# Cornell-RelaxML/QuIP

Hardware: NVIDIA H100
Metric: tokens/sec 2-bit Llama-2-7B (per-layer eval path, seq 2048) (higher is better)
Workload: dtype f16

## Files before the change

quip_b200/csrc/api.cu:

```cuda
#include <stdarg.h>
#include <string.h>

#include <vector>

#include "common.cuh"

namespace quip {

static thread_local char g_err[512] = "";
std::atomic<int64_t> g_launches{0};

void set_error(const char* fmt, ...) {
  va_list ap;
  va_start(ap, fmt);
  vsnprintf(g_err, sizeof(g_err), fmt, ap);
  va_end(ap);
}

int qgemm_skinny(const QuipLinearDesc* d, const __half* x, const __half* bias, __half* z, int M, int ksplit,
                 float* part, int* counters, cudaStream_t s);
int skinny_pick_ksplit(int N, int K, int rows_per_cta, int M);
size_t skinny_workspace_bytes(int N, int M, int ksplit);
int qgemv(const QuipLinearDesc* d, const __half* x, const __half* bias, __half* z, int M, cudaStream_t s);
bool qgemv_fits(int K, int M, int bits);
int qgemm_tc(const QuipLinearDesc* d, const __half* x, const float* xsum, const __half* bias, __half* z, int M,
             cudaStream_t s);

extern int g_gather_rows, g_pass_min_tiles, g_fewtok;
extern int g_fewtok_max_m;
bool side_fused_ok(const QuipSide* sd, int n);
int side_fused(const QuipSide* sd, const __half* in, __half* out, int64_t M, const int32_t* in_idx, const float* in_scale,
               const int32_t* out_idx, const __half* out_bias, float* xsum, cudaStream_t s);
bool pass_fewtok_ok(const QuipPass* ps, int64_t M, int n);
int pass_fewtok(const QuipPass* ps, const __half* in, __half* out, int64_t M, int n, const int32_t* in_idx,
                const float* in_scale, const int32_t* out_inv, const __half* out_bias, cudaStream_t s);
extern int g_gv_rbc, g_gv_persist, g_gv_int, g_gv_tma, g_gv_cw, g_gv_stream;
bool side_fewtok_ok(const QuipSide* sd, int n, int64_t M);
int side_fewtok(const QuipSide* sd, const __half* in, __half* out, int64_t M, int n, const int32_t* in_idx,
                const float* in_scale, const int32_t* out_inv, const __half* out_bias, cudaStream_t s);

static int g_side_fused = 1;
static int g_pdl = 1;
static int g_use_gemv = 1;
static int g_sk_ksplit = 0;
static int g_side_fewtok = 0;

int launch_pdl(const void* kern, dim3 grid, dim3 block, size_t smem, cudaStream_t s, void** args) {
  cudaLaunchConfig_t cfg = {};
  cfg.gridDim = grid;
  cfg.blockDim = block;
  cfg.dynamicSmemBytes = smem;
  cfg.stream = s;
  cudaLaunchAttribute attr[1];
  attr[0].id = cudaLaunchAttributeProgrammaticStreamSerialization;
  attr[0].val.programmaticStreamSerializationAllowed = 1;
  cfg.attrs = attr;
  cfg.numAttrs = g_pdl ? 1 : 0;
  cudaError_t e = cudaLaunchKernelExC(&cfg, kern, args);
  if (e != cudaSuccess) {
    cudaGetLastError();
    set_error("kernel launch failed: %s", cudaGetErrorString(e));
    return QUIP_ERR_CUDA;
  }
  return QUIP_OK;
}

constexpr size_t WS_HEADER = 16 * 1024;
constexpr int SKINNY_MAX_M = 32;

static size_t align_up(size_t v, size_t a) { return (v + a - 1) / a * a; }

struct WsPlan {
  size_t xsum, bufA, bufB, zbuf, bufC, part, total;
};
// ... 12 lines not shown
  p.bufB = off; if (v_on) off += xk;
  p.zbuf = off; if (u_on) off += xn;
  p.bufC = off; if (u_on) off += xn;
  p.part = off;
  const int mc = M <= SKINNY_MAX_M ? (int)M : SKINNY_MAX_M;
  off += align_up(skinny_workspace_bytes(d->N, mc, skinny_pick_ksplit(d->N, d->K, 64, mc)), 256);
  p.total = off;
  return p;
}

static int check_desc(const QuipLinearDesc* d) {
  QUIP_CHECK_ARG(d != nullptr, "null descriptor");
  QUIP_CHECK_ARG(d->bits >= 2 && d->bits <= 4, "bits must be 2, 3 or 4 (got %d)", d->bits);
  QUIP_CHECK_ARG(d->K > 0 && d->K % 128 == 0, "K=%d must be a positive multiple of 128", d->K);
  QUIP_CHECK_ARG(d->N > 0 && d->N % 16 == 0, "N=%d must be a positive multiple of 16", d->N);
  QUIP_CHECK_ARG(d->qweight && d->scales && d->zeros, "qweight / scales / zeros must be set");
  QUIP_CHECK_ARG(d->V.n == 0 || d->V.n == d->K, "V side size %d != K %d", d->V.n, d->K);
  QUIP_CHECK_ARG(d->U.n == 0 || d->U.n == d->N, "U side size %d != N %d", d->U.n, d->N);
  QUIP_CHECK_ARG(d->V.npass >= 0 && d->V.npass <= 2 && d->U.npass >= 0 && d->U.npass <= 2, "npass must be 0..2");
  return QUIP_OK;
}

struct TimedLaunch {
  cudaEvent_t e0, e1;
  int path;
  double flops, bytes;
};
static bool g_timing = false;
static std::vector<TimedLaunch> g_timed;
static std::vector<TimedLaunch> g_pool;
constexpr size_t TIMED_MAX = 1 << 16;

static int run_qgemm_untimed(const QuipLinearDesc* d, const __half* x2, const float* xsum, const __half* bias,
                             __half* z, int64_t M, int path, unsigned char* ws, const WsPlan& p, cudaStream_t s);

static int run_qgemm(const QuipLinearDesc* d, const __half* x2, const float* xsum, const __half* bias, __half* z,
                     int64_t M, int path, unsigned char* ws, const WsPlan& p, cudaStream_t s) {
  if (path == 0)
    path = M <= SKINNY_MAX_M ? 1 : 2;
  if (!g_timing || g_timed.size() >= TIMED_MAX) return run_qgemm_untimed(d, x2, xsum, bias, z, M, path, ws, p, s);
  TimedLaunch t;
  if (!g_pool.empty()) {
    t = g_pool.back();
    g_pool.pop_back();
  } else {
    QUIP_CUDA(cudaEventCreate(&t.e0));
    QUIP_CUDA(cudaEventCreate(&t.e1));
  }
  t.path = path;
  t.flops = 2.0 * (double)M * d->N * d->K;
  t.bytes = (double)d->N * d->K * d->bits / 8.0 + 2.0 * (double)M * (d->K + d->N);
  QUIP_CUDA(cudaEventRecord(t.e0, s));
  int e = run_qgemm_untimed(d, x2, xsum, bias, z, M, path, ws, p, s);
  QUIP_CUDA(cudaEventRecord(t.e1, s));
  g_timed.push_back(t);
  return e;
}

static int run_qgemm_untimed(const QuipLinearDesc* d, const __half* x2, const float* xsum, const __half* bias,
                             __half* z, int64_t M, int path, unsigned char* ws, const WsPlan& p, cudaStream_t s) {
  if (path == 1) {
    for (int64_t m0 = 0; m0 < M; m0 += SKINNY_MAX_M) {
      int mc = (int)((M - m0) < SKINNY_MAX_M ? (M - m0) : SKINNY_MAX_M);
      if (g_use_gemv && qgemv_fits(d->K, mc, d->bits)) {
        if (int e = qgemv(d, x2 + m0 * d->K, bias, z + m0 * d->N, mc, s)) return e;
        continue;
      }
      int ksplit = skinny_pick_ksplit(d->N, d->K, 64, mc);
      if (g_sk_ksplit > 0 && g_sk_ksplit < ksplit) ksplit = g_sk_ksplit;
      if (int e = qgemm_skinny(d, x2 + m0 * d->K, bias, z + m0 * d->N, mc, ksplit,
                               reinterpret_cast<float*>(ws + p.part), reinterpret_cast<int*>(ws), s))
        return e;
    }
    return QUIP_OK;
  }
  const bool need_xsum = !(d->flags & QUIP_FLAG_SYMMETRIC);
  QUIP_CHECK_ARG(!need_xsum || xsum, "asymmetric grid needs the row sums of x");
  return qgemm_tc(d, x2, xsum, bias, z, (int)M, s);
}

}

using namespace quip;

extern "C" const char* quip_last_error(void) { return g_err; }
extern "C" int quip_abi_version(void) { return QUIP_ABI_VERSION; }
extern "C" int64_t quip_launch_count(void) { return g_launches.load(); }

extern "C" int quip_config(const char* key, int value) {
  QUIP_CHECK_ARG(key != nullptr, "null key");
  if (!strcmp(key, "side_fused")) { g_side_fused = value; return QUIP_OK; }
  if (!strcmp(key, "side_fewtok")) { g_side_fewtok = value; return QUIP_OK; }
  if (!strcmp(key, "pdl")) { g_pdl = value; return QUIP_OK; }
  if (!strcmp(key, "fewtok")) { g_fewtok = value; return QUIP_OK; }
  if (!strcmp(key, "fewtok_max_m")) {
    QUIP_CHECK_ARG(value >= 8 && value <= 32, "quip_config: fewtok_max_m must be in 8..32");
    g_fewtok_max_m = value;
    return QUIP_OK;
  }
  if (!strcmp(key, "gemv")) { g_use_gemv = value; return QUIP_OK; }
  if (!strcmp(key, "gv_rbc")) { g_gv_rbc = value; return QUIP_OK; }
  if (!strcmp(key, "gv_stream")) { g_gv_stream = value; return QUIP_OK; }
  if (!strcmp(key, "gv_cw")) { g_gv_cw = value; return QUIP_OK; }
  if (!strcmp(key, "gv_tma")) { g_gv_tma = value; return QUIP_OK; }
  if (!strcmp(key, "gv_int")) { g_gv_int = value; return QUIP_OK; }
  if (!strcmp(key, "gv_persist")) { g_gv_persist = value; return QUIP_OK; }
  if (!strcmp(key, "gather_rows")) { g_gather_rows = value; return QUIP_OK; }
  if (!strcmp(key, "sk_ksplit")) { g_sk_ksplit = value; return QUIP_OK; }
  if (!strcmp(key, "pass_min_tiles")) { g_pass_min_tiles = value > 0 ? value : 1; return QUIP_OK; }
  set_error("quip_config: unknown key '%s'", key);
  return QUIP_ERR_ARG;
}

extern "C" int quip_timing_enable(int on) {
  g_timing = on != 0;
  return QUIP_OK;
}
extern "C" int quip_timing_reset(void) {
  for (auto& t : g_timed) g_pool.push_back(t);
  g_timed.clear();
  return QUIP_OK;
}
extern "C" int quip_timing_read(int path, double* total_ms, int64_t* launches, double* flops, double* bytes) {
  double ms = 0, fl = 0, by = 0;
// ... 1 lines not shown
  for (auto& t : g_timed) {
    if (t.path != path) continue;
    QUIP_CUDA(cudaEventSynchronize(t.e1));
    float dt = 0.f;
    QUIP_CUDA(cudaEventElapsedTime(&dt, t.e0, t.e1));
    ms += dt; fl += t.flops; by += t.bytes; ++n;
  }
  if (total_ms) *total_ms = ms;
  if (launches) *launches = n;
  if (flops) *flops = fl;
  if (bytes) *bytes = by;
  return QUIP_OK;
}

extern "C" int quip_qlinear_workspace_bytes(const QuipLinearDesc* d, int64_t M, size_t* out) {
  if (int e = check_desc(d)) return e;
  QUIP_CHECK_ARG(out && M > 0, "bad arguments");
  *out = plan_ws(d, M).total;
  return QUIP_OK;
}

extern "C" int quip_qgemm(const QuipLinearDesc* d, const void* x2, const float* xsum, const void* bias, void* z,
                          int64_t M, int path, void* workspace, size_t workspace_bytes, void* stream) {
  if (int e = check_desc(d)) return e;
  QUIP_CHECK_ARG(x2 && z && M > 0 && M < (1ll << 31), "bad arguments");
  WsPlan p = plan_ws(d, M);
  QUIP_CHECK_ARG(path >= 0 && path <= 2, "path must be 0 (auto), 1 (few-token kernels) or 2 (tensor-core GEMM)");
  if (path == 1 || (path == 0 && M <= SKINNY_MAX_M)) {
    if (!workspace || workspace_bytes < p.total) {
      set_error("workspace too small: need %zu bytes, have %zu", p.total, workspace_bytes);
      return QUIP_ERR_WORKSPACE;
    }
  }
  return run_qgemm(d, (const __half*)x2, xsum, (const __half*)bias, (__half*)z, M, path, (unsigned char*)workspace, p,
                   (cudaStream_t)stream);
}

extern "C" int quip_qlinear_forward(const QuipLinearDesc* d, const void* x_, void* y_, int64_t M, void* workspace,
                                    size_t workspace_bytes, void* stream) {
  if (int e = check_desc(d)) return e;
  QUIP_CHECK_ARG(x_ && y_ && M > 0 && M < (1ll << 31), "bad arguments");
  cudaStream_t s = (cudaStream_t)stream;
  WsPlan p = plan_ws(d, M);
  if (!workspace || workspace_bytes < p.total) {
    set_error("workspace too small: need %zu bytes, have %zu", p.total, workspace_bytes);
    return QUIP_ERR_WORKSPACE;
  }
  unsigned char* ws = (unsigned char*)workspace;
  const __half* x = (const __half*)x_;
  __half* y = (__half*)y_;
  __half* bufA = (__half*)(ws + p.bufA);
  __half* bufB = (__half*)(ws + p.bufB);
  __half* zbuf = (__half*)(ws + p.zbuf);
  __half* bufC = (__half*)(ws + p.bufC);
  float* xsum = (float*)(ws + p.xsum);
  const int K = d->K, N = d->N;

  const __half* cur = x;
  const int vpass = d->V.n ? d->V.npass : 0;
  const bool need_xsum = !(d->flags & QUIP_FLAG_SYMMETRIC) && M > SKINNY_MAX_M;
  bool have_xsum = false;
  if (g_fewtok && g_side_fewtok && vpass == 2 && side_fewtok_ok(&d->V, K, M)) {
    if (int e = side_fewtok(&d->V, x, bufA, M, K, d->V.idx, d->inv_scale, nullptr, nullptr, s)) return e;
    cur = bufA;
  } else if (g_side_fused && M > g_fewtok_max_m && vpass == 2 && side_fused_ok(&d->V, K)) {
    if (int e = side_fused(&d->V, x, bufA, M, d->V.idx, d->inv_scale, nullptr, nullptr, need_xsum ? xsum : nullptr, s)) return e;
    cur = bufA;
    have_xsum = need_xsum;
  } else {
    const bool fuse_in = g_fewtok && M <= g_fewtok_max_m && vpass > 0 && d->V.pass[0].p <= 128 && pass_fewtok_ok(&d->V.pass[0], M, K);
    if ((d->V.idx || d->inv_scale) && !fuse_in) {
      if (int e = quip_gather(cur, bufA, M, K, d->V.n ? d->V.idx : nullptr, d->inv_scale, nullptr, stream)) return e;
      cur = bufA;
    }
    for (int i = 0; i < vpass; ++i) {
      __half* dst = (cur == bufA) ? bufB : bufA;
      if (i == 0 && fuse_in) {
        if (int e = pass_fewtok(&d->V.pass[0], cur, dst, M, K, d->V.idx, d->inv_scale, nullptr, nullptr, s)) return e;
      } else if (int e = quip_rot_pass(&d->V.pass[i], cur, dst, M, K, 0, stream)) {
        return e;
      }
      cur = dst;
    }
  }
  const __half* x2 = cur;

  const bool u_on = side_on(d->U);
  if (need_xsum && !have_xsum)
    if (int e = quip_rowsum(x2, xsum, M, K, stream)) return e;
  __half* zdst = u_on ? zbuf : y;
  if (int e = run_qgemm(d, x2, xsum, u_on ? nullptr : (const __half*)d->bias, zdst, M, 0, ws, p, s)) return e;
  if (!u_on) return QUIP_OK;

  if (g_fewtok && g_side_fewtok && d->U.npass == 2 && (!d->U.idx || d->U.inv_idx) && side_fewtok_ok(&d->U, N, M))
    return side_fewtok(&d->U, zbuf, y, M, N, nullptr, nullptr, d->U.inv_idx, (const __half*)d->bias, s);
  if (g_side_fused && M > g_fewtok_max_m && d->U.npass == 2 && side_fused_ok(&d->U, N))
    return side_fused(&d->U, zbuf, y, M, nullptr, nullptr, d->U.idx, (const __half*)d->bias, nullptr, s);
  const __half* zc = zbuf;
  const int np = d->U.npass;
  bool tail_gather = d->U.idx || d->bias;
  const bool fuse_out = tail_gather && g_fewtok && M <= g_fewtok_max_m && np > 0 && (!d->U.idx || d->U.inv_idx) &&
                        pass_fewtok_ok(&d->U.pass[np - 1], M, N);
  if (fuse_out) tail_gather = false;
  for (int i = 0; i < np; ++i) {
    __half* dst = (i == np - 1 && !tail_gather) ? y : ((zc == zbuf) ? bufC : zbuf);
    if (i == np - 1 && fuse_out) {
      if (int e = pass_fewtok(&d->U.pass[i], zc, dst, M, N, nullptr, nullptr, d->U.inv_idx, (const __half*)d->bias, s)) return e;
    } else if (int e = quip_rot_pass(&d->U.pass[i], zc, dst, M, N, 0, stream)) {
      return e;
    }
    zc = dst;
  }
  if (tail_gather) return quip_gather(zc, y, M, N, d->U.idx, nullptr, d->bias, stream);
  return QUIP_OK;
}
```

quip_b200/csrc/qgemm_tc.cu:

```cuda
#include "tc_common.cuh"

namespace quip {

constexpr int TC_SMEM_MAX = 227 * 1024;

template <int BITS, int BN, bool DENSE>
struct TcCfg {
  static constexpr int A_BYTES = DENSE ? TC_BM * TC_BK * 2 : (TC_BM / SB_ROWS) * sb_words(BITS) * 4;
  static constexpr int B_BYTES = BN * TC_BK * 2;
  static constexpr int STAGE_BYTES = A_BYTES + B_BYTES;
  static constexpr int EPI_HALVES = BN * 72 > 64 * (BN + 8) ? BN * 72 : 64 * (BN + 8);
  static constexpr int EPI_BYTES = 2 * EPI_HALVES * 2;
  static constexpr int STAGES_FIT = (TC_SMEM_MAX - EPI_BYTES - 1024 - 256) / STAGE_BYTES;
  static constexpr int STAGES = STAGES_FIT < 16 ? STAGES_FIT : 16;
  static constexpr size_t SMEM = (size_t)STAGES * STAGE_BYTES + 1024  + 256  + EPI_BYTES;
  static_assert(STAGE_BYTES % 1024 == 0 && 2 * STAGES * 8 <= 256, "stage layout");
};

template <int BITS, int BN, bool DENSE>
__global__ void __launch_bounds__(TC_THREADS, 1)
qgemm_tc_kernel(const __grid_constant__ CUtensorMap tmap_x, const __grid_constant__ CUtensorMap tmap_a,
                const float* __restrict__ scales, const float* __restrict__ zeros, const __half* __restrict__ bias,
                const float* __restrict__ xsum, __half* __restrict__ z, int M, int K, int N, int symmetric, int nblk,
                int shared_factor) {
  using C = TcCfg<BITS, BN, DENSE>;
  extern __shared__ unsigned char smem_raw[];
  const uint32_t smem_base = (smem_u32(smem_raw) + 1023u) & ~1023u;
  unsigned char* smem_gen = smem_raw + (smem_base - smem_u32(smem_raw));
  uint64_t* bars = reinterpret_cast<uint64_t*>(smem_gen + (size_t)C::STAGES * C::STAGE_BYTES);
  uint64_t* full = bars;
  uint64_t* empty = bars + C::STAGES;
  __half* epi = reinterpret_cast<__half*>(smem_gen + (size_t)C::STAGES * C::STAGE_BYTES + 256);

  const int warp = threadIdx.x >> 5, lane = threadIdx.x & 31;
  const int tiles_n = DENSE ? (N + BN - 1) / BN : (N + TC_BM - 1) / TC_BM;
  const int tiles_m = DENSE ? (M + TC_BM - 1) / TC_BM : (M + BN - 1) / BN;
  const int per_blk = tiles_n * tiles_m;
  const int num_tiles = per_blk * nblk;
  const int KB = (K + TC_BK - 1) / TC_BK;
  const int64_t ldz = (int64_t)N * nblk;
  constexpr int TMA_WARP = TC_CONSUMER_WARPS;

  if (warp == TMA_WARP && lane == 0) {
    asm volatile("prefetch.tensormap [%0];" ::"l"(&tmap_x) : "memory");
    asm volatile("prefetch.tensormap [%0];" ::"l"(&tmap_a) : "memory");
    for (int s = 0; s < C::STAGES; ++s) {
      mbar_init(&full[s], 1);
      mbar_init(&empty[s], TC_CONSUMER_WARPS);
    }
    asm volatile("fence.mbarrier_init.release.cluster;" ::: "memory");
  }
  __syncthreads();

  if (warp == TMA_WARP) {
    if (lane == 0) {
      int s = 0;
      uint32_t ph = 0;
// ... 21 lines not shown
    const int wg = warp >> 2, wtid = threadIdx.x & 127;
    const int frow = (warp & 3) * 16 + (lane >> 2);
    const int fcol = (lane & 3) * 2;
    __half* eb = epi + wg * C::EPI_HALVES;
    float acc[BN / 2];
#pragma unroll
    for (int j = 0; j < BN / 2; ++j) acc[j] = 0.f;
    int s = 0;
    uint32_t ph = 0;
    auto advance = [&]() { if (++s == C::STAGES) { s = 0; ph ^= 1u; } };
    auto release = [&](int st) {
      __syncwarp();
      if (lane == 0) mbar_arrive(&empty[st]);
    };
    for (int tile = blockIdx.x; tile < num_tiles; tile += gridDim.x) {
      const int blk = tile / per_blk, rr = tile % per_blk;
      int prev = 0;
      const int n_base = (rr % tiles_n) * TC_BM + wg * 64, m0 = (rr / tiles_n) * BN;
      float Pn[2], Rn[2], bn[2];
      if constexpr (!DENSE) {
#pragma unroll
        for (int h = 0; h < 2; ++h) {
          const int n = n_base + frow + 8 * h;
          Pn[h] = 1.f; Rn[h] = 0.f; bn[h] = 0.f;
          if (n < N) {
            const float sc = scales[n];
            Pn[h] = sc * (float)(1 << BITS);
            if (!symmetric) Rn[h] = sc * (0.5f * (float)((1 << BITS) - 1)) - zeros[n];
            if (bias) bn[h] = __half2float(bias[n]);
          }
        }
        if (!symmetric && wtid < BN / 32 && m0 + 32 * wtid < M)
          asm volatile("prefetch.global.L1 [%0];" ::"l"(xsum + m0 + 32 * wtid));
      }
      if constexpr (DENSE) {
        for (int kb = 0; kb < KB; ++kb) {
          mbar_wait(&full[s], ph);
          const uint32_t a_addr = smem_base + (uint32_t)(s * C::STAGE_BYTES);
          const uint64_t adesc = make_sw128_desc(a_addr + (uint32_t)(wg * 64 * 128));
          const uint64_t bdesc = make_sw128_desc(a_addr + C::A_BYTES);
          wgmma_fence();
#pragma unroll
          for (int k = 0; k < TC_BK / 16; ++k)
            wgmma_f16_ss<BN>(acc, adesc + (uint64_t)(2 * k), bdesc + (uint64_t)(2 * k), (kb | k) ? 1 : 0);
          wgmma_commit();
          wgmma_wait<1>();
          if (kb > 0) release(prev);
          prev = s;
          advance();
        }
      } else {
        const int g = lane >> 2, t = lane & 3;
        const uint32_t row_off = (uint32_t)(warp * sb_words(BITS) * 4);
        uint32_t w[row_words(BITS)];
        uint32_t fa[2][16];
        auto issue = [&](const uint32_t (&f)[16], int first) {
          const uint64_t bdesc = make_sw128_desc(smem_base + (uint32_t)(s * C::STAGE_BYTES) + C::A_BYTES);
          wgmma_fence();
#pragma unroll
          for (int k = 0; k < TC_BK / 16; ++k)
            wgmma_f16_rs<BN>(acc, &f[4 * k], bdesc + (uint64_t)(2 * k), (first && k == 0) ? 0 : 1);
          wgmma_commit();
        };
        auto load_words = [&]() {
          mbar_wait(&full[s], ph);
          tc_load_row_words<BITS>(smem_base + (uint32_t)(s * C::STAGE_BYTES) + row_off, g, w);
// ... 21 lines not shown
          prev = s;
          advance();
          if (ksb + 1 < KSB) {
            load_words();
            frag_natural<BITS, 0, 0>(w, t, &fa[0][0]);
            frag_natural<BITS, 0, 1>(w, t, &fa[0][4]);
            frag_natural<BITS, 1, 0>(w, t, &fa[0][8]);
            frag_natural<BITS, 1, 1>(w, t, &fa[0][12]);
          }
        }
      }
      wgmma_wait<0>();
      wgmma_fence_regs(acc);
      release(prev);

      if constexpr (DENSE) {
        constexpr int EP = BN + 8;
#pragma unroll
        for (int j = 0; j < BN / 2; j += 2) {
          const int r = frow + ((j & 2) ? 8 : 0), c = 8 * (j >> 2) + fcol;
          *reinterpret_cast<__half2*>(&eb[r * EP + c]) = __floats2half2_rn(acc[j], acc[j + 1]);
        }
        asm volatile("bar.sync %0, 128;" ::"r"(1 + wg) : "memory");
        const int m_base = (rr / tiles_n) * TC_BM + wg * 64, i0 = (rr % tiles_n) * BN;
        for (int idx = wtid; idx < 64 * (BN / 8); idx += 128) {
          const int r = idx / (BN / 8), v = idx % (BN / 8);
          const int m = m_base + r, i = i0 + 8 * v;
          if (m < M && i < N)
            *reinterpret_cast<uint4*>(z + (int64_t)m * ldz + (int64_t)blk * N + i) =
                *reinterpret_cast<const uint4*>(&eb[r * EP + 8 * v]);
        }
      } else {
        constexpr int EP = 72;
#pragma unroll
        for (int j = 0; j < BN / 2; ++j) {
          const int h = (j >> 1) & 1, c = 8 * (j >> 2) + fcol + (j & 1), m = m0 + c;
          float v = Pn[h] * acc[j] + bn[h];
          if (!symmetric) v += Rn[h] * (m < M ? __ldg(&xsum[m]) : 0.f);
          eb[c * EP + frow + 8 * h] = __float2half_rn(v);
        }
        asm volatile("bar.sync %0, 128;" ::"r"(1 + wg) : "memory");
        for (int idx = wtid; idx < BN * 8; idx += 128) {
          const int c = idx >> 3, v = idx & 7;
          const int m = m0 + c, n = n_base + 8 * v;
          if (m < M && n < N)
            *reinterpret_cast<uint4*>(z + (int64_t)m * ldz + n) = *reinterpret_cast<const uint4*>(&eb[c * EP + 8 * v]);
        }
      }
      asm volatile("bar.sync %0, 128;" ::"r"(1 + wg) : "memory");
    }
  }
}

typedef CUresult (*PFN_encodeTiled)(CUtensorMap*, CUtensorMapDataType, cuuint32_t, void*, const cuuint64_t*,
                                    const cuuint64_t*, const cuuint32_t*, const cuuint32_t*, CUtensorMapInterleave,
                                    CUtensorMapSwizzle, CUtensorMapL2promotion, CUtensorMapFloatOOBfill);

static PFN_encodeTiled get_encode() {
  static PFN_encodeTiled fn = nullptr;
  if (!fn) {
    void* p = nullptr;
    cudaDriverEntryPointQueryResult qres;
    if (cudaGetDriverEntryPoint("cuTensorMapEncodeTiled", &p, cudaEnableDefault, &qres) == cudaSuccess &&
        qres == cudaDriverEntryPointSuccess)
      fn = (PFN_encodeTiled)p;
  }
  return fn;
}

static int g_num_sms = 0;

int num_sms() {
// ... 19 lines not shown
  CUresult r = enc(tmap, CU_TENSOR_MAP_DATA_TYPE_FLOAT16, 2, (void*)x, dims, strides, box, estr,
                   CU_TENSOR_MAP_INTERLEAVE_NONE, CU_TENSOR_MAP_SWIZZLE_128B, CU_TENSOR_MAP_L2_PROMOTION_L2_256B,
                   CU_TENSOR_MAP_FLOAT_OOB_FILL_NONE);
  if (r != CUDA_SUCCESS) {
    set_error("cuTensorMapEncodeTiled failed with CUresult %d (ptr=%p rows=%lld cols=%lld)", (int)r, x,
              (long long)rows, (long long)cols);
    return QUIP_ERR_CUDA;
  }
  return QUIP_OK;
}

static int make_words_map(CUtensorMap* tmap, const QuipLinearDesc* d) {
  PFN_encodeTiled enc = get_encode();
  if (!enc) {
    set_error("cuTensorMapEncodeTiled is not available from the driver");
    return QUIP_ERR_CUDA;
  }
  const int sbw = sb_words(d->bits);
  cuuint64_t dims[2] = {(cuuint64_t)(d->K / SB_K) * sbw, (cuuint64_t)(d->N / SB_ROWS)};
  cuuint64_t strides[1] = {dims[0] * sizeof(uint32_t)};
  cuuint32_t box[2] = {(cuuint32_t)sbw, (cuuint32_t)(TC_BM / SB_ROWS)};
  cuuint32_t estr[2] = {1, 1};
  CUresult r = enc(tmap, CU_TENSOR_MAP_DATA_TYPE_UINT32, 2, (void*)d->qweight, dims, strides, box, estr,
                   CU_TENSOR_MAP_INTERLEAVE_NONE, CU_TENSOR_MAP_SWIZZLE_NONE, CU_TENSOR_MAP_L2_PROMOTION_L2_256B,
                   CU_TENSOR_MAP_FLOAT_OOB_FILL_NONE);
  if (r != CUDA_SUCCESS) {
    set_error("cuTensorMapEncodeTiled (packed words) failed with CUresult %d (N=%d K=%d bits=%d)", (int)r, d->N, d->K,
              d->bits);
    return QUIP_ERR_CUDA;
  }
  return QUIP_OK;
}

template <int BITS, int BN>
static int launch_tc(const QuipLinearDesc* d, const __half* x, const float* xsum, const __half* bias, __half* z,
                     int M, cudaStream_t s) {
  using C = TcCfg<BITS, BN, false>;
  CUtensorMap tmx, tmq;
  if (int e = make_act_map(&tmx, x, M, d->K, BN)) return e;
  if (int e = make_words_map(&tmq, d)) return e;
  auto kern = qgemm_tc_kernel<BITS, BN, false>;
  QUIP_CUDA(cudaFuncSetAttribute(kern, cudaFuncAttributeMaxDynamicSharedMemorySize, (int)C::SMEM));
  int tiles = ceil_div(d->N, TC_BM) * ceil_div(M, BN);
  int grid = tiles < num_sms() ? tiles : num_sms();
  kern<<<grid, TC_THREADS, C::SMEM, s>>>(tmx, tmq, d->scales, d->zeros, bias, xsum, z, M, d->K, d->N,
                                         (d->flags & QUIP_FLAG_SYMMETRIC) ? 1 : 0, 1, 0);
  QUIP_LAUNCHED("qgemm_tc_kernel");
  return QUIP_OK;
}

template <int BN>
static int launch_tc_dense(const QuipPass* ps, const __half* in, __half* out, int M, int n, cudaStream_t s) {
  using C = TcCfg<2, BN, true>;
  PFN_encodeTiled enc = get_encode();
  CUtensorMap tmx, tma;
  if (int e = make_act_map(&tmx, in, M, n, TC_BM)) return e;
  const int p = ps->p;
  cuuint64_t dims[3] = {(cuuint64_t)p, (cuuint64_t)p, (cuuint64_t)(ps->shared ? 1 : ps->nblk)};
  cuuint64_t strides[2] = {(cuuint64_t)p * sizeof(__half), (cuuint64_t)p * p * sizeof(__half)};
  cuuint32_t box[3] = {(cuuint32_t)TC_BK, (cuuint32_t)BN, 1};
  cuuint32_t estr[3] = {1, 1, 1};
  CUresult r = enc(&tma, CU_TENSOR_MAP_DATA_TYPE_FLOAT16, 3, (void*)ps->factors, dims, strides, box, estr,
                   CU_TENSOR_MAP_INTERLEAVE_NONE, CU_TENSOR_MAP_SWIZZLE_128B, CU_TENSOR_MAP_L2_PROMOTION_L2_256B,
                   CU_TENSOR_MAP_FLOAT_OOB_FILL_NONE);
  if (r != CUDA_SUCCESS) {
    set_error("cuTensorMapEncodeTiled (factors) failed with CUresult %d (p=%d nblk=%d)", (int)r, p, ps->nblk);
    return QUIP_ERR_CUDA;
  }
  auto kern = qgemm_tc_kernel<2, BN, true>;
  QUIP_CUDA(cudaFuncSetAttribute(kern, cudaFuncAttributeMaxDynamicSharedMemorySize, (int)C::SMEM));
  int tiles = ceil_div(p, BN) * ceil_div(M, TC_BM) * ps->nblk;
  int grid = tiles < num_sms() ? tiles : num_sms();
  kern<<<grid, TC_THREADS, C::SMEM, s>>>(tmx, tma, nullptr, nullptr, nullptr, nullptr, out, M, p, p, 1,
                                         ps->nblk, ps->shared ? 1 : 0);
  QUIP_LAUNCHED("qgemm_tc_kernel<dense>");
  return QUIP_OK;
}

int pass_big_tc(const QuipPass* ps, const __half* in, __half* out, int64_t M, int n, cudaStream_t s) {
  QUIP_CHECK_ARG(!ps->strided && ps->p % 8 == 0 && n % 8 == 0, "tensor-core pass needs contiguous blocks, p %% 8 == 0");
  QUIP_CHECK_ARG((((uintptr_t)in | (uintptr_t)out | (uintptr_t)ps->factors) & 15) == 0, "tensor-core pass: unaligned pointer");
  return launch_tc_dense<128>(ps, in, out, (int)M, n, s);
}

int qgemm_tc(const QuipLinearDesc* d, const __half* x, const float* xsum, const __half* bias, __half* z, int M,
             cudaStream_t s) {
  QUIP_CHECK_ARG((((uintptr_t)x | (uintptr_t)d->qweight) & 15) == 0,
                 "tensor-core path needs 16-byte aligned activations and packed words");
  const bool wide = M > 64;
#define QUIP_TC(B)                                                            \
  if (d->bits == B)                                                           \
    return wide ? launch_tc<B, 128>(d, x, xsum, bias, z, M, s) : launch_tc<B, 64>(d, x, xsum, bias, z, M, s);
  QUIP_TC(2) QUIP_TC(3) QUIP_TC(4)
#undef QUIP_TC
  set_error("tensor-core kernel: unsupported bits=%d", d->bits);
  return QUIP_ERR_UNSUPPORTED;
}

}
```

quip_b200/csrc/rot_side.cu:

```cuda
#include "common.cuh"

namespace quip {

constexpr int SD_TOK = 16;
constexpr int SD_WARPS = 16;

template <int PA, int PB>
struct SideCfg {
  static constexpr int N = PA * PB;
  static constexpr int SU = PB + 2;
  static constexpr int R0 = (PA / 2) * SU;
  static constexpr int R = R0 + ((8 - R0 % 32) + 32) % 32;
  static constexpr size_t T_BYTES = (size_t)SD_TOK * R * 4;
  static constexpr size_t S_BYTES = (size_t)8 * N * sizeof(__half);
  static constexpr size_t SMEM = T_BYTES + S_BYTES + SD_TOK * SD_WARPS * sizeof(float);
};

__device__ __forceinline__ uint32_t pack_h2(float lo, float hi) {
  __half2 h = __floats2half2_rn(lo, hi);
  return *reinterpret_cast<uint32_t*>(&h);
}

template <int P>
__device__ __forceinline__ uint4 frag_load(const uint4* __restrict__ blk, int nt, int j, int lane) {
// ... 111 lines not shown
#pragma unroll
        for (int q = 0; q < G; ++q) {
          float c0[4] = {0.f, 0.f, 0.f, 0.f}, c1[4] = {0.f, 0.f, 0.f, 0.f};
#pragma unroll
          for (int j = 0; j < J; ++j) {
            const uint32_t p0[2] = {bf0[q][j].x, bf0[q][j].y}, p1[2] = {bf0[q][j].z, bf0[q][j].w};
            const uint32_t r0[2] = {bf1[q][j].x, bf1[q][j].y}, r1[2] = {bf1[q][j].z, bf1[q][j].w};
            mma16816(c0, a0[2 * j], p0);
            mma16816(c0, a0[2 * j + 1], p1);
            mma16816(c1, a1[2 * j], r0);
            mma16816(c1, a1[2 * j + 1], r1);
          }
          uint32_t* w = T + g * C::R + u * C::SU + 8 * (grp * G + q) + 2 * t;
          w[0] = pack_h2(c0[0], c1[0]);
          w[1] = pack_h2(c0[1], c1[1]);
          w[8 * C::R] = pack_h2(c0[2], c1[2]);
          w[8 * C::R + 1] = pack_h2(c0[3], c1[3]);
        }
      }
#pragma unroll
      for (int q = 0; q < G; ++q)
#pragma unroll
        for (int j = 0; j < J; ++j) { bf0[q][j] = nx0[q][j]; bf1[q][j] = nx1[q][j]; }
    }
  }
};

template <int PA, int PB>
__device__ __forceinline__ int half_index(int l) {
  const int a = l / PB, b = l - a * PB;
  return 2 * ((a >> 1) * SideCfg<PA, PB>::SU + b) + (a & 1);
}

template <int PA, int PB>
__global__ void __launch_bounds__(SD_WARPS * 32)
side_fused_kernel(const __half* __restrict__ in, __half* __restrict__ out, int64_t M, const int32_t* __restrict__ in_idx,
                  const float* __restrict__ in_scale, const int32_t* __restrict__ out_idx,
                  const __half* __restrict__ out_bias, const uint4* __restrict__ F_col, int col_shared,
                  const uint4* __restrict__ F_row, int row_shared, int col_first, float* __restrict__ xsum) {
  using C = SideCfg<PA, PB>;
  constexpr int N = C::N, NTH = SD_WARPS * 32;
  extern __shared__ __align__(16) unsigned char smem_raw[];
  uint32_t* T = reinterpret_cast<uint32_t*>(smem_raw);
  __half* T16 = reinterpret_cast<__half*>(smem_raw);
  __half* S = reinterpret_cast<__half*>(smem_raw + C::T_BYTES);
  float* wsum = reinterpret_cast<float*>(smem_raw + C::T_BYTES + C::S_BYTES);
  const int tid = threadIdx.x, warp = tid >> 5, lane = tid & 31;
  const int64_t m0 = (int64_t)blockIdx.x * SD_TOK;
  const int nr = (int)((M - m0) < SD_TOK ? (M - m0) : SD_TOK);

  ColPass<PA, PB> colp;
  RowPass<PA, PB> rowp;
  if (col_first) colp.prefetch(F_col, col_shared, warp, lane);
  else rowp.prefetch(F_row, row_shared, warp, lane);

  if (in_idx || in_scale) {
    constexpr int WPT = (N / 2 + NTH - 1) / NTH;
    int src0[WPT], src1[WPT];
    float sc0[WPT], sc1[WPT];
#pragma unroll
    for (int i = 0; i < WPT; ++i) {
      const int w = tid + i * NTH;
      src0[i] = src1[i] = 0; sc0[i] = sc1[i] = 1.f;
      if (w < N / 2) {
        const int u = w / PB, b = w - u * PB;
        const int l0 = (2 * u) * PB + b, l1 = l0 + PB;
        src0[i] = in_idx ? __ldg(in_idx + l0) : l0;
        src1[i] = in_idx ? __ldg(in_idx + l1) : l1;
        if (in_scale) { sc0[i] = __ldg(in_scale + src0[i]); sc1[i] = __ldg(in_scale + src1[i]); }
      }
    }
    constexpr int CHT = (N / 8 + NTH - 1) / NTH;
    uint4 v[8][CHT];
    auto request = [&](int r0) {
#pragma unroll
      for (int r = 0; r < 8; ++r)
#pragma unroll
        for (int i = 0; i < CHT; ++i) {
          const int c = tid + i * NTH;
          v[r][i] = make_uint4(0u, 0u, 0u, 0u);
          if (c < N / 8 && r0 + r < nr) v[r][i] = ldg_nc_v4(in + (m0 + r0 + r) * N + 8 * c);
        }
    };
    auto park = [&]() {
#pragma unroll
      for (int r = 0; r < 8; ++r)
// ... 33 lines not shown
    constexpr int ITEMS = SD_TOK * (PA / 2) * (PB / 8), PER = (ITEMS + NTH - 1) / NTH, BATCH = PER < 4 ? PER : 4;
#pragma unroll 1
    for (int i0 = 0; i0 < PER; i0 += BATCH) {
      uint4 lo[BATCH], hi[BATCH];
#pragma unroll
      for (int i = 0; i < BATCH; ++i) {
        const int c = tid + (i0 + i) * NTH;
        const int r = c / ((PA / 2) * (PB / 8)), rem = c - r * ((PA / 2) * (PB / 8));
        const int u = rem / (PB / 8), b0 = (rem - u * (PB / 8)) * 8;
        lo[i] = hi[i] = make_uint4(0u, 0u, 0u, 0u);
        if (i0 + i < PER && c < ITEMS && r < nr) {
          lo[i] = ldg_nc_v4(in + (m0 + r) * N + (size_t)(2 * u) * PB + b0);
          hi[i] = ldg_nc_v4(in + (m0 + r) * N + (size_t)(2 * u + 1) * PB + b0);
        }
      }
#pragma unroll
      for (int i = 0; i < BATCH; ++i) {
        const int c = tid + (i0 + i) * NTH;
        if (i0 + i < PER && c < ITEMS) {
          const int r = c / ((PA / 2) * (PB / 8)), rem = c - r * ((PA / 2) * (PB / 8));
          const int u = rem / (PB / 8), b0 = (rem - u * (PB / 8)) * 8;
          uint32_t* w = T + r * C::R + u * C::SU + b0;
          w[0] = __byte_perm(lo[i].x, hi[i].x, 0x5410); w[1] = __byte_perm(lo[i].x, hi[i].x, 0x7632);
          w[2] = __byte_perm(lo[i].y, hi[i].y, 0x5410); w[3] = __byte_perm(lo[i].y, hi[i].y, 0x7632);
          w[4] = __byte_perm(lo[i].z, hi[i].z, 0x5410); w[5] = __byte_perm(lo[i].z, hi[i].z, 0x7632);
          w[6] = __byte_perm(lo[i].w, hi[i].w, 0x5410); w[7] = __byte_perm(lo[i].w, hi[i].w, 0x7632);
        }
      }
    }
    __syncthreads();
  }

  if (col_first) {
    colp.run(T, F_col, col_shared, warp, lane);
    rowp.prefetch(F_row, row_shared, warp, lane);
    __syncthreads();
    rowp.run(T, F_row, row_shared, warp, lane);
  } else {
    rowp.run(T, F_row, row_shared, warp, lane);
    colp.prefetch(F_col, col_shared, warp, lane);
    __syncthreads();
    colp.run(T, F_col, col_shared, warp, lane);
  }
  __syncthreads();

  if (out_idx || out_bias) {
    constexpr int CPT = (N / 8 + NTH - 1) / NTH;
    int hidx[CPT][8];
    float bs[CPT][8];
#pragma unroll
    for (int i = 0; i < CPT; ++i) {
      const int c = tid + i * NTH;
#pragma unroll
      for (int e = 0; e < 8; ++e) {
        hidx[i][e] = 0; bs[i][e] = 0.f;
        if (c < N / 8) {
          const int j = 8 * c + e;
          hidx[i][e] = half_index<PA, PB>(out_idx ? __ldg(out_idx + j) : j);
          if (out_bias) bs[i][e] = __half2float(__ldg(out_bias + j));
        }
      }
    }
    for (int r = 0; r < nr; ++r) {
      const __half* row = T16 + (size_t)r * 2 * C::R;
#pragma unroll
      for (int i = 0; i < CPT; ++i) {
        const int c = tid + i * NTH;
        if (c < N / 8) {
          __align__(16) __half v[8];
#pragma unroll
          for (int e = 0; e < 8; ++e) v[e] = __float2half_rn(__half2float(row[hidx[i][e]]) + bs[i][e]);
          *reinterpret_cast<uint4*>(out + (m0 + r) * N + 8 * c) = *reinterpret_cast<const uint4*>(v);
        }
      }
// ... 2 lines not shown
    constexpr int CPR = PA * (PB / 8);
    for (int r = 0; r < nr; ++r) {
      float s = 0.f;
      for (int c = tid; c < CPR; c += NTH) {
        const int a = c / (PB / 8), b0 = (c - a * (PB / 8)) * 8;
        const uint32_t* w = T + r * C::R + (a >> 1) * C::SU + b0;
        const uint32_t sel = (a & 1) ? 0x7632u : 0x5410u;
        uint4 v;
        v.x = __byte_perm(w[0], w[1], sel); v.y = __byte_perm(w[2], w[3], sel);
        v.z = __byte_perm(w[4], w[5], sel); v.w = __byte_perm(w[6], w[7], sel);
        *reinterpret_cast<uint4*>(out + (m0 + r) * N + (size_t)a * PB + b0) = v;
        const __half2* h = reinterpret_cast<const __half2*>(&v);
#pragma unroll
        for (int e = 0; e < 4; ++e) { const float2 f = __half22float2(h[e]); s += f.x + f.y; }
      }
      if (xsum) {
#pragma unroll
        for (int o = 16; o; o >>= 1) s += __shfl_xor_sync(0xffffffffu, s, o);
        if (lane == 0) wsum[r * SD_WARPS + warp] = s;
      }
    }
    if (xsum) {
      __syncthreads();
      if (tid < nr) {
        float s = 0.f;
#pragma unroll
        for (int w = 0; w < SD_WARPS; ++w) s += wsum[tid * SD_WARPS + w];
        xsum[m0 + tid] = s;
      }
    }
  }
}

template <int PA, int PB>
static int launch_side(const __half* in, __half* out, int64_t M, const int32_t* in_idx, const float* in_scale,
                       const int32_t* out_idx, const __half* out_bias, const QuipPass* col, const QuipPass* row,
                       int col_first, float* xsum, cudaStream_t s) {
  using C = SideCfg<PA, PB>;
  auto kern = side_fused_kernel<PA, PB>;
  static bool attr_done[64] = {false};
  int dev = 0;
  QUIP_CUDA(cudaGetDevice(&dev));
  dev &= 63;
  if (!attr_done[dev]) {
    QUIP_CUDA(cudaFuncSetAttribute(kern, cudaFuncAttributeMaxDynamicSharedMemorySize, (int)C::SMEM));
    attr_done[dev] = true;
  }
  kern<<<(unsigned)ceil_div(M, SD_TOK), SD_WARPS * 32, C::SMEM, s>>>(
      in, out, M, in_idx, in_scale, out_idx, out_bias, (const uint4*)col->factors_frag, col->shared,
      (const uint4*)row->factors_frag, row->shared, col_first, xsum);
  QUIP_LAUNCHED("side_fused_kernel");
  return QUIP_OK;
}

bool side_fused_ok(const QuipSide* sd, int n) {
  if (sd->n != n || sd->npass != 2) return false;
  const QuipPass& p0 = sd->pass[0];
  const QuipPass& p1 = sd->pass[1];
  const QuipPass* col = p0.strided ? &p0 : (p1.strided ? &p1 : nullptr);
  const QuipPass* row = p0.strided ? &p1 : &p0;
  if (!col || row->strided) return false;
  if (col->p != row->nblk || col->nblk != row->p) return false;
  if (!col->factors_frag || !row->factors_frag) return false;
  const int PA = col->p, PB = row->p;
  return (PA == 64 && PB == 64) || (PA == 32 && PB == 64) || (PA == 64 && PB == 32);
}

int side_fused(const QuipSide* sd, const __half* in, __half* out, int64_t M, const int32_t* in_idx, const float* in_scale,
               const int32_t* out_idx, const __half* out_bias, float* xsum, cudaStream_t s) {
  const QuipPass& p0 = sd->pass[0];
  const QuipPass* col = p0.strided ? &sd->pass[0] : &sd->pass[1];
  const QuipPass* row = p0.strided ? &sd->pass[1] : &sd->pass[0];
  const int col_first = p0.strided ? 1 : 0;
  const int PA = col->p, PB = row->p;
  if (PA == 64 && PB == 64) return launch_side<64, 64>(in, out, M, in_idx, in_scale, out_idx, out_bias, col, row, col_first, xsum, s);
  if (PA == 32 && PB == 64) return launch_side<32, 64>(in, out, M, in_idx, in_scale, out_idx, out_bias, col, row, col_first, xsum, s);
  if (PA == 64 && PB == 32) return launch_side<64, 32>(in, out, M, in_idx, in_scale, out_idx, out_bias, col, row, col_first, xsum, s);
  set_error("fused side: unsupported block sizes %d x %d", PA, PB);
  return QUIP_ERR_UNSUPPORTED;
}

}
```

Measured before the change: 26200.

## Fold first U-side rotation pass into tensor-core GEMM epilogue

For large M with a two-pass fused U side, the first (contiguous 64-block) U rotation pass now runs inside the wgmma GEMM epilogue. The dequantized tile is staged in swizzled shared memory and multiplied by the block factors with a register-sourced wgmma. The side kernel is then launched in a one-pass mode that skips that pass. This removes one full pass of rotation math and smem work from the side kernel, at the cost of a longer GEMM epilogue, extra registers and an added fp16 rounding before the fold.

```diff
diff --git a/quip_b200/csrc/api.cu b/quip_b200/csrc/api.cu
--- a/quip_b200/csrc/api.cu
+++ b/quip_b200/csrc/api.cu
@@ -24,13 +24,14 @@
 int qgemv(const QuipLinearDesc* d, const __half* x, const __half* bias, __half* z, int M, cudaStream_t s);
 bool qgemv_fits(int K, int M, int bits);
 int qgemm_tc(const QuipLinearDesc* d, const __half* x, const float* xsum, const __half* bias, __half* z, int M,
-             cudaStream_t s);
+             const QuipPass* ufold, cudaStream_t s);
+bool qgemm_tc_fold_ok(const QuipPass* ps, int N);
 
 extern int g_gather_rows, g_pass_min_tiles, g_fewtok;
 extern int g_fewtok_max_m;
 bool side_fused_ok(const QuipSide* sd, int n);
 int side_fused(const QuipSide* sd, const __half* in, __half* out, int64_t M, const int32_t* in_idx, const float* in_scale,
-               const int32_t* out_idx, const __half* out_bias, float* xsum, cudaStream_t s);
+               const int32_t* out_idx, const __half* out_bias, float* xsum, int skip_first, cudaStream_t s);
 bool pass_fewtok_ok(const QuipPass* ps, int64_t M, int n);
 int pass_fewtok(const QuipPass* ps, const __half* in, __half* out, int64_t M, int n, const int32_t* in_idx,
                 const float* in_scale, const int32_t* out_inv, const __half* out_bias, cudaStream_t s);
@@ -40,6 +41,7 @@
                 const float* in_scale, const int32_t* out_inv, const __half* out_bias, cudaStream_t s);
 
 static int g_side_fused = 1;
+static int g_gemm_ufold = 1;
 static int g_pdl = 1;
 static int g_use_gemv = 1;
 static int g_sk_ksplit = 0;
@@ -118,13 +120,14 @@
 constexpr size_t TIMED_MAX = 1 << 16;
 
 static int run_qgemm_untimed(const QuipLinearDesc* d, const __half* x2, const float* xsum, const __half* bias,
-                             __half* z, int64_t M, int path, unsigned char* ws, const WsPlan& p, cudaStream_t s);
+                             __half* z, int64_t M, int path, const QuipPass* ufold, unsigned char* ws, const WsPlan& p,
+                             cudaStream_t s);
 
 static int run_qgemm(const QuipLinearDesc* d, const __half* x2, const float* xsum, const __half* bias, __half* z,
-                     int64_t M, int path, unsigned char* ws, const WsPlan& p, cudaStream_t s) {
+                     int64_t M, int path, const QuipPass* ufold, unsigned char* ws, const WsPlan& p, cudaStream_t s) {
   if (path == 0)
     path = M <= SKINNY_MAX_M ? 1 : 2;
-  if (!g_timing || g_timed.size() >= TIMED_MAX) return run_qgemm_untimed(d, x2, xsum, bias, z, M, path, ws, p, s);
+  if (!g_timing || g_timed.size() >= TIMED_MAX) return run_qgemm_untimed(d, x2, xsum, bias, z, M, path, ufold, ws, p, s);
   TimedLaunch t;
   if (!g_pool.empty()) {
     t = g_pool.back();
@@ -137,14 +140,16 @@
   t.flops = 2.0 * (double)M * d->N * d->K;
   t.bytes = (double)d->N * d->K * d->bits / 8.0 + 2.0 * (double)M * (d->K + d->N);
   QUIP_CUDA(cudaEventRecord(t.e0, s));
-  int e = run_qgemm_untimed(d, x2, xsum, bias, z, M, path, ws, p, s);
+  int e = run_qgemm_untimed(d, x2, xsum, bias, z, M, path, ufold, ws, p, s);
   QUIP_CUDA(cudaEventRecord(t.e1, s));
   g_timed.push_back(t);
   return e;
 }
 
 static int run_qgemm_untimed(const QuipLinearDesc* d, const __half* x2, const float* xsum, const __half* bias,
-                             __half* z, int64_t M, int path, unsigned char* ws, const WsPlan& p, cudaStream_t s) {
+                             __half* z, int64_t M, int path, const QuipPass* ufold, unsigned char* ws, const WsPlan& p,
+                             cudaStream_t s) {
+  QUIP_CHECK_ARG(!ufold || path == 2, "the epilogue U pass runs in the wgmma kernel only");
   if (path == 1) {
     for (int64_t m0 = 0; m0 < M; m0 += SKINNY_MAX_M) {
       int mc = (int)((M - m0) < SKINNY_MAX_M ? (M - m0) : SKINNY_MAX_M);
@@ -162,7 +167,7 @@
   }
   const bool need_xsum = !(d->flags & QUIP_FLAG_SYMMETRIC);
   QUIP_CHECK_ARG(!need_xsum || xsum, "asymmetric grid needs the row sums of x");
-  return qgemm_tc(d, x2, xsum, bias, z, (int)M, s);
+  return qgemm_tc(d, x2, xsum, bias, z, (int)M, ufold, s);
 }
 
 }
@@ -176,6 +181,7 @@
 extern "C" int quip_config(const char* key, int value) {
   QUIP_CHECK_ARG(key != nullptr, "null key");
   if (!strcmp(key, "side_fused")) { g_side_fused = value; return QUIP_OK; }
+  if (!strcmp(key, "gemm_ufold")) { g_gemm_ufold = value; return QUIP_OK; }
   if (!strcmp(key, "side_fewtok")) { g_side_fewtok = value; return QUIP_OK; }
   if (!strcmp(key, "pdl")) { g_pdl = value; return QUIP_OK; }
   if (!strcmp(key, "fewtok")) { g_fewtok = value; return QUIP_OK; }
@@ -243,8 +249,8 @@
       return QUIP_ERR_WORKSPACE;
     }
   }
-  return run_qgemm(d, (const __half*)x2, xsum, (const __half*)bias, (__half*)z, M, path, (unsigned char*)workspace, p,
-                   (cudaStream_t)stream);
+  return run_qgemm(d, (const __half*)x2, xsum, (const __half*)bias, (__half*)z, M, path, nullptr,
+                   (unsigned char*)workspace, p, (cudaStream_t)stream);
 }
 
 extern "C" int quip_qlinear_forward(const QuipLinearDesc* d, const void* x_, void* y_, int64_t M, void* workspace,
@@ -275,7 +281,7 @@
     if (int e = side_fewtok(&d->V, x, bufA, M, K, d->V.idx, d->inv_scale, nullptr, nullptr, s)) return e;
     cur = bufA;
   } else if (g_side_fused && M > g_fewtok_max_m && vpass == 2 && side_fused_ok(&d->V, K)) {
-    if (int e = side_fused(&d->V, x, bufA, M, d->V.idx, d->inv_scale, nullptr, nullptr, need_xsum ? xsum : nullptr, s)) return e;
+    if (int e = side_fused(&d->V, x, bufA, M, d->V.idx, d->inv_scale, nullptr, nullptr, need_xsum ? xsum : nullptr, 0, s)) return e;
     cur = bufA;
     have_xsum = need_xsum;
   } else {
@@ -300,13 +306,17 @@
   if (need_xsum && !have_xsum)
     if (int e = quip_rowsum(x2, xsum, M, K, stream)) return e;
   __half* zdst = u_on ? zbuf : y;
-  if (int e = run_qgemm(d, x2, xsum, u_on ? nullptr : (const __half*)d->bias, zdst, M, 0, ws, p, s)) return e;
+  const bool side_one = g_side_fused && M > g_fewtok_max_m && d->U.npass == 2 && side_fused_ok(&d->U, N);
+  const bool ufold = side_one && g_gemm_ufold && M > SKINNY_MAX_M && qgemm_tc_fold_ok(&d->U.pass[0], N);
+  if (int e = run_qgemm(d, x2, xsum, u_on ? nullptr : (const __half*)d->bias, zdst, M, 0, ufold ? &d->U.pass[0] : nullptr,
+                        ws, p, s))
+    return e;
   if (!u_on) return QUIP_OK;
 
   if (g_fewtok && g_side_fewtok && d->U.npass == 2 && (!d->U.idx || d->U.inv_idx) && side_fewtok_ok(&d->U, N, M))
     return side_fewtok(&d->U, zbuf, y, M, N, nullptr, nullptr, d->U.inv_idx, (const __half*)d->bias, s);
-  if (g_side_fused && M > g_fewtok_max_m && d->U.npass == 2 && side_fused_ok(&d->U, N))
-    return side_fused(&d->U, zbuf, y, M, nullptr, nullptr, d->U.idx, (const __half*)d->bias, nullptr, s);
+  if (side_one)
+    return side_fused(&d->U, zbuf, y, M, nullptr, nullptr, d->U.idx, (const __half*)d->bias, nullptr, ufold ? 1 : 0, s);
   const __half* zc = zbuf;
   const int np = d->U.npass;
   bool tail_gather = d->U.idx || d->bias;
diff --git a/quip_b200/csrc/qgemm_tc.cu b/quip_b200/csrc/qgemm_tc.cu
--- a/quip_b200/csrc/qgemm_tc.cu
+++ b/quip_b200/csrc/qgemm_tc.cu
@@ -17,12 +17,13 @@
   static_assert(STAGE_BYTES % 1024 == 0 && 2 * STAGES * 8 <= 256, "stage layout");
 };
 
-template <int BITS, int BN, bool DENSE>
+template <int BITS, int BN, bool DENSE, bool FOLD = false>
 __global__ void __launch_bounds__(TC_THREADS, 1)
 qgemm_tc_kernel(const __grid_constant__ CUtensorMap tmap_x, const __grid_constant__ CUtensorMap tmap_a,
                 const float* __restrict__ scales, const float* __restrict__ zeros, const __half* __restrict__ bias,
                 const float* __restrict__ xsum, __half* __restrict__ z, int M, int K, int N, int symmetric, int nblk,
-                int shared_factor) {
+                int shared_factor, const uint4* __restrict__ ufold) {
+  static_assert(!(DENSE && FOLD), "the epilogue pass belongs to the packed GEMM");
   using C = TcCfg<BITS, BN, DENSE>;
   extern __shared__ unsigned char smem_raw[];
   const uint32_t smem_base = (smem_u32(smem_raw) + 1023u) & ~1023u;
@@ -110,6 +111,14 @@
         }
         if (!symmetric && wtid < BN / 32 && m0 + 32 * wtid < M)
           asm volatile("prefetch.global.L1 [%0];" ::"l"(xsum + m0 + 32 * wtid));
+      }
+      const uint4* Fb = nullptr;
+      if constexpr (FOLD) {
+        Fb = ufold + (size_t)(shared_factor ? 0 : n_base / 64) * (64 * 64 / 8);
+        if (n_base < N)
+#pragma unroll
+          for (int i = 0; i < 4; ++i)
+            asm volatile("prefetch.global.L1 [%0];" ::"l"(Fb + (2 * (warp & 3) * 2 + i) * 32 + lane));
       }
       if constexpr (DENSE) {
         for (int kb = 0; kb < KB; ++kb) {
@@ -197,12 +206,54 @@
         }
       } else {
         constexpr int EP = 72;
-#pragma unroll
-        for (int j = 0; j < BN / 2; ++j) {
-          const int h = (j >> 1) & 1, c = 8 * (j >> 2) + fcol + (j & 1), m = m0 + c;
-          float v = Pn[h] * acc[j] + bn[h];
-          if (!symmetric) v += Rn[h] * (m < M ? __ldg(&xsum[m]) : 0.f);
-          eb[c * EP + frow + 8 * h] = __float2half_rn(v);
+        if constexpr (FOLD) {
+          uint32_t fu[16];
+          if (n_base < N) {
+#pragma unroll
+            for (int j = 0; j < 2; ++j) {
+              const uint4 lo = __ldg(Fb + ((2 * (warp & 3)) * 2 + j) * 32 + lane);
+              const uint4 hi = __ldg(Fb + ((2 * (warp & 3) + 1) * 2 + j) * 32 + lane);
+              uint32_t* f = &fu[8 * j];
+              f[0] = lo.x; f[1] = hi.x; f[2] = lo.y; f[3] = hi.y;
+              f[4] = lo.z; f[5] = hi.z; f[6] = lo.w; f[7] = hi.w;
+            }
+          } else {
+#pragma unroll
+            for (int i = 0; i < 16; ++i) fu[i] = 0u;
+          }
+          static_assert(C::EPI_BYTES / 2 % 1024 == 0 && C::EPI_BYTES / 2 >= 768 + BN * 128, "fold tile in eb");
+          const uint32_t sw = (smem_u32(eb) + 1023u) & ~1023u;
+#pragma unroll
+          for (int j = 0; j < BN / 2; ++j) {
+            const int h = (j >> 1) & 1, c = 8 * (j >> 2) + fcol + (j & 1), m = m0 + c, r = frow + 8 * h;
+            float v = Pn[h] * acc[j] + bn[h];
+            if (!symmetric) v += Rn[h] * (m < M ? __ldg(&xsum[m]) : 0.f);
+            const __half hv = __float2half_rn(v);
+            asm volatile("st.shared.b16 [%0], %1;" ::"r"(sw + (uint32_t)(c * 128 + (((r >> 3) ^ (c & 7)) << 4) + (r & 7) * 2)),
+                         "h"(*reinterpret_cast<const unsigned short*>(&hv)) : "memory");
+          }
+          asm volatile("fence.proxy.async.shared::cta;" ::: "memory");
+          asm volatile("bar.sync %0, 128;" ::"r"(1 + wg) : "memory");
+          wgmma_fence();
+#pragma unroll
+          for (int ks = 0; ks < 4; ++ks) wgmma_f16_rs<BN>(acc, &fu[4 * ks], make_sw128_desc(sw) + (uint64_t)(2 * ks), ks);
+          wgmma_commit();
+          wgmma_wait<0>();
+          wgmma_fence_regs(acc);
+          asm volatile("bar.sync %0, 128;" ::"r"(1 + wg) : "memory");
+#pragma unroll
+          for (int j = 0; j < BN / 2; ++j) {
+            const int h = (j >> 1) & 1, c = 8 * (j >> 2) + fcol + (j & 1);
+            eb[c * EP + frow + 8 * h] = __float2half_rn(acc[j]);
+          }
+        } else {
+#pragma unroll
+          for (int j = 0; j < BN / 2; ++j) {
+            const int h = (j >> 1) & 1, c = 8 * (j >> 2) + fcol + (j & 1), m = m0 + c;
+            float v = Pn[h] * acc[j] + bn[h];
+            if (!symmetric) v += Rn[h] * (m < M ? __ldg(&xsum[m]) : 0.f);
+            eb[c * EP + frow + 8 * h] = __float2half_rn(v);
+          }
         }
         asm volatile("bar.sync %0, 128;" ::"r"(1 + wg) : "memory");
         for (int idx = wtid; idx < BN * 8; idx += 128) {
@@ -288,19 +339,20 @@
   return QUIP_OK;
 }
 
-template <int BITS, int BN>
+template <int BITS, int BN, bool FOLD>
 static int launch_tc(const QuipLinearDesc* d, const __half* x, const float* xsum, const __half* bias, __half* z,
-                     int M, cudaStream_t s) {
+                     int M, const QuipPass* ufold, cudaStream_t s) {
   using C = TcCfg<BITS, BN, false>;
   CUtensorMap tmx, tmq;
   if (int e = make_act_map(&tmx, x, M, d->K, BN)) return e;
   if (int e = make_words_map(&tmq, d)) return e;
-  auto kern = qgemm_tc_kernel<BITS, BN, false>;
+  auto kern = qgemm_tc_kernel<BITS, BN, false, FOLD>;
   QUIP_CUDA(cudaFuncSetAttribute(kern, cudaFuncAttributeMaxDynamicSharedMemorySize, (int)C::SMEM));
   int tiles = ceil_div(d->N, TC_BM) * ceil_div(M, BN);
   int grid = tiles < num_sms() ? tiles : num_sms();
   kern<<<grid, TC_THREADS, C::SMEM, s>>>(tmx, tmq, d->scales, d->zeros, bias, xsum, z, M, d->K, d->N,
-                                         (d->flags & QUIP_FLAG_SYMMETRIC) ? 1 : 0, 1, 0);
+                                         (d->flags & QUIP_FLAG_SYMMETRIC) ? 1 : 0, 1, FOLD ? ufold->shared : 0,
+                                         FOLD ? (const uint4*)ufold->factors_frag : nullptr);
   QUIP_LAUNCHED("qgemm_tc_kernel");
   return QUIP_OK;
 }
@@ -328,7 +380,7 @@
   int tiles = ceil_div(p, BN) * ceil_div(M, TC_BM) * ps->nblk;
   int grid = tiles < num_sms() ? tiles : num_sms();
   kern<<<grid, TC_THREADS, C::SMEM, s>>>(tmx, tma, nullptr, nullptr, nullptr, nullptr, out, M, p, p, 1,
-                                         ps->nblk, ps->shared ? 1 : 0);
+                                         ps->nblk, ps->shared ? 1 : 0, nullptr);
   QUIP_LAUNCHED("qgemm_tc_kernel<dense>");
   return QUIP_OK;
 }
@@ -339,14 +391,25 @@
   return launch_tc_dense<128>(ps, in, out, (int)M, n, s);
 }
 
+bool qgemm_tc_fold_ok(const QuipPass* ps, int N) {
+  return ps && !ps->strided && ps->p == 64 && ps->nblk * 64 == N && ps->factors_frag &&
+         ((uintptr_t)ps->factors_frag & 15) == 0;
+}
+
 int qgemm_tc(const QuipLinearDesc* d, const __half* x, const float* xsum, const __half* bias, __half* z, int M,
-             cudaStream_t s) {
+             const QuipPass* ufold, cudaStream_t s) {
   QUIP_CHECK_ARG((((uintptr_t)x | (uintptr_t)d->qweight) & 15) == 0,
                  "tensor-core path needs 16-byte aligned activations and packed words");
+  QUIP_CHECK_ARG(!ufold || qgemm_tc_fold_ok(ufold, d->N), "epilogue pass: contiguous 64-blocks covering N only");
   const bool wide = M > 64;
-#define QUIP_TC(B)                                                            \
-  if (d->bits == B)                                                           \
-    return wide ? launch_tc<B, 128>(d, x, xsum, bias, z, M, s) : launch_tc<B, 64>(d, x, xsum, bias, z, M, s);
+#define QUIP_TC(B)                                                                                       \
+  if (d->bits == B) {                                                                                    \
+    if (ufold)                                                                                           \
+      return wide ? launch_tc<B, 128, true>(d, x, xsum, bias, z, M, ufold, s)                            \
+                  : launch_tc<B, 64, true>(d, x, xsum, bias, z, M, ufold, s);                            \
+    return wide ? launch_tc<B, 128, false>(d, x, xsum, bias, z, M, nullptr, s)                           \
+                : launch_tc<B, 64, false>(d, x, xsum, bias, z, M, nullptr, s);                           \
+  }
   QUIP_TC(2) QUIP_TC(3) QUIP_TC(4)
 #undef QUIP_TC
   set_error("tensor-core kernel: unsupported bits=%d", d->bits);
diff --git a/quip_b200/csrc/rot_side.cu b/quip_b200/csrc/rot_side.cu
--- a/quip_b200/csrc/rot_side.cu
+++ b/quip_b200/csrc/rot_side.cu
@@ -167,7 +167,7 @@
   return 2 * ((a >> 1) * SideCfg<PA, PB>::SU + b) + (a & 1);
 }
 
-template <int PA, int PB>
+template <int PA, int PB, bool ONE_PASS>
 __global__ void __launch_bounds__(SD_WARPS * 32)
 side_fused_kernel(const __half* __restrict__ in, __half* __restrict__ out, int64_t M, const int32_t* __restrict__ in_idx,
                   const float* __restrict__ in_scale, const int32_t* __restrict__ out_idx,
@@ -186,7 +186,7 @@
 
   ColPass<PA, PB> colp;
   RowPass<PA, PB> rowp;
-  if (col_first) colp.prefetch(F_col, col_shared, warp, lane);
+  if (col_first != ONE_PASS) colp.prefetch(F_col, col_shared, warp, lane);
   else rowp.prefetch(F_row, row_shared, warp, lane);
 
   if (in_idx || in_scale) {
@@ -286,14 +286,18 @@
   }
 
   if (col_first) {
-    colp.run(T, F_col, col_shared, warp, lane);
-    rowp.prefetch(F_row, row_shared, warp, lane);
-    __syncthreads();
+    if (!ONE_PASS) {
+      colp.run(T, F_col, col_shared, warp, lane);
+      rowp.prefetch(F_row, row_shared, warp, lane);
+      __syncthreads();
+    }
     rowp.run(T, F_row, row_shared, warp, lane);
   } else {
-    rowp.run(T, F_row, row_shared, warp, lane);
-    colp.prefetch(F_col, col_shared, warp, lane);
-    __syncthreads();
+    if (!ONE_PASS) {
+      rowp.run(T, F_row, row_shared, warp, lane);
+      colp.prefetch(F_col, col_shared, warp, lane);
+      __syncthreads();
+    }
     colp.run(T, F_col, col_shared, warp, lane);
   }
   __syncthreads();
@@ -362,12 +366,12 @@
   }
 }
 
-template <int PA, int PB>
+template <int PA, int PB, bool ONE_PASS>
 static int launch_side(const __half* in, __half* out, int64_t M, const int32_t* in_idx, const float* in_scale,
                        const int32_t* out_idx, const __half* out_bias, const QuipPass* col, const QuipPass* row,
                        int col_first, float* xsum, cudaStream_t s) {
   using C = SideCfg<PA, PB>;
-  auto kern = side_fused_kernel<PA, PB>;
+  auto kern = side_fused_kernel<PA, PB, ONE_PASS>;
   static bool attr_done[64] = {false};
   int dev = 0;
   QUIP_CUDA(cudaGetDevice(&dev));
@@ -397,15 +401,18 @@
 }
 
 int side_fused(const QuipSide* sd, const __half* in, __half* out, int64_t M, const int32_t* in_idx, const float* in_scale,
-               const int32_t* out_idx, const __half* out_bias, float* xsum, cudaStream_t s) {
+               const int32_t* out_idx, const __half* out_bias, float* xsum, int skip_first, cudaStream_t s) {
   const QuipPass& p0 = sd->pass[0];
   const QuipPass* col = p0.strided ? &sd->pass[0] : &sd->pass[1];
   const QuipPass* row = p0.strided ? &sd->pass[1] : &sd->pass[0];
   const int col_first = p0.strided ? 1 : 0;
   const int PA = col->p, PB = row->p;
-  if (PA == 64 && PB == 64) return launch_side<64, 64>(in, out, M, in_idx, in_scale, out_idx, out_bias, col, row, col_first, xsum, s);
-  if (PA == 32 && PB == 64) return launch_side<32, 64>(in, out, M, in_idx, in_scale, out_idx, out_bias, col, row, col_first, xsum, s);
-  if (PA == 64 && PB == 32) return launch_side<64, 32>(in, out, M, in_idx, in_scale, out_idx, out_bias, col, row, col_first, xsum, s);
+#define QUIP_SIDE(A, B)                                                                                                 \
+  if (PA == A && PB == B)                                                                                              \
+    return skip_first ? launch_side<A, B, true>(in, out, M, in_idx, in_scale, out_idx, out_bias, col, row, col_first, xsum, s) \
+                      : launch_side<A, B, false>(in, out, M, in_idx, in_scale, out_idx, out_bias, col, row, col_first, xsum, s);
+  QUIP_SIDE(64, 64) QUIP_SIDE(32, 64) QUIP_SIDE(64, 32)
+#undef QUIP_SIDE
   set_error("fused side: unsupported block sizes %d x %d", PA, PB);
   return QUIP_ERR_UNSUPPORTED;
 }
```

Result: faster. 26490 (median of 6 runs) (+1.1%).
